# nem0/LumixEngine

Hardware: AMD Instinct MI355X
Metric: entities_culled_per_sec (higher is better)
Workload: dtype f32; 1 GPU; BASELINE config 2: 10000000 static entities per GPU (sparse, cube +-15000), 1 frustum (fov 60, 16:9, near 0.1, far 10000), cull + compaction; entities_per_gpu=10000000, frusta=1, repetitions=1

## Files before the change

lumixengine_amd/build.py:

```python
from __future__ import annotations

import os
import shutil
import subprocess
import sys
from concurrent.futures import ThreadPoolExecutor

PKG = os.path.dirname(os.path.abspath(__file__))
ROOT = os.path.dirname(PKG)
CSRC = os.path.join(PKG, "csrc")
OBJ = os.path.join(PKG, "build")
LIB = os.path.join(PKG, "liblumix_mi355.so")
SOURCES = ["cull_kernels.hip", "xform_kernels.hip", "skin_kernels.hip", "lmx_capi_ctx.hip", "lmx_capi_cull.hip", "lmx_capi_cull_set.hip", "lmx_capi_cull_async.hip", "lmx_capi_cull_results.hip", "lmx_capi_world.hip",
           "lmx_capi_skin.hip", "lmx_capi_exchange.hip", "keys_kernels.hip", "lmx_capi_keys.hip", "anim_kernels.hip", "lmx_capi_anim.hip", "im_kernels.hip", "lmx_capi_im.hip", "draw_kernels.hip", "lmx_capi_draw.hip", "pose_kernels.hip", "lmx_capi_poses.hip", "cluster_kernels.hip", "lmx_capi_clusters.hip", "ray_kernels.hip", "lmx_capi_rays.hip", "ray_scene_kernels.hip", "lmx_capi_rays_scene.hip",
           "lmx_frustum.cpp", "lmx_cluster_planes.cpp", "lmx_world_blob.cpp"]
HEADERS = [os.path.join(CSRC, "lmx_math.h"), os.path.join(CSRC, "lmx_kernels.h"), os.path.join(CSRC, "lmx_cull_layout.h"), os.path.join(CSRC, "lmx_context.h"), os.path.join(CSRC, "lmx_cull_host.h"), os.path.join(CSRC, "lmx_im.h"), os.path.join(CSRC, "lmx_entity_tr.h"), os.path.join(CSRC, "lmx_ray_math.h"), os.path.join(ROOT, "include", "lumix_mi355.h"),
           os.path.join(ROOT, "include", "lmx_types.h")]
FLAGS = ["--offload-arch=gfx950", "-O3", "-std=c++17", "-ffp-contract=off", "-fPIC", "-fvisibility=hidden", "-Wall", "-Wno-unused-function",
         "-I" + os.path.join(ROOT, "include"), "-I" + CSRC] + os.environ.get("LMX_HIPCC_EXTRA", "").split()


def hipcc() -> str:
    exe = shutil.which("hipcc") or "/opt/rocm/bin/hipcc"
    if not os.path.exists(exe):
        raise RuntimeError("hipcc not found: the gfx950 extension cannot be built")
    return exe


def _stale(target: str, deps) -> bool:
    if not os.path.exists(target):
        return True
    t = os.path.getmtime(target)
    return any(os.path.getmtime(d) > t for d in deps)


def _compile(src: str) -> str:
    path = os.path.join(CSRC, src)
    obj = os.path.join(OBJ, os.path.splitext(src)[0] + ".o")
    if _stale(obj, [path] + HEADERS):
        cmd = [hipcc()] + FLAGS + (["-x", "hip"] if src.endswith(".hip") else []) + ["-c", path, "-o", obj]
        r = subprocess.run(cmd, capture_output=True, text=True)
        if r.returncode != 0:
            raise RuntimeError(f"hipcc failed for {src}:\n{r.stdout}\n{r.stderr}")
    return obj


def build(force: bool = False) -> str:
    os.makedirs(OBJ, exist_ok=True)
    if force:
        for f in os.listdir(OBJ):
            os.remove(os.path.join(OBJ, f))
        if os.path.exists(LIB):
            os.remove(LIB)
    with ThreadPoolExecutor(max_workers=len(SOURCES)) as ex:
        objs = list(ex.map(_compile, SOURCES))
# ... 11 lines not shown
```

lumixengine_amd/csrc/cull_kernels.hip:

```cpp
#include <algorithm>
#include <cstddef>
#include <cstdlib>

#include "lmx_kernels.h"
#include <type_traits>

#include <hip/hip_ext.h>

namespace lmx {

namespace {

__device__ __forceinline__ uint32_t lane_id() { return __builtin_amdgcn_mbcnt_hi(~0u, __builtin_amdgcn_mbcnt_lo(~0u, 0u)); }
__device__ __forceinline__ uint32_t mbcnt64(uint64_t mask) {
	return __builtin_amdgcn_mbcnt_hi((uint32_t)(mask >> 32), __builtin_amdgcn_mbcnt_lo((uint32_t)mask, 0u));
}
typedef uint32_t u32x4_a4 __attribute__((ext_vector_type(4), aligned(4)));
__device__ __forceinline__ float readlane_f(float v, int lane) { return __uint_as_float(__builtin_amdgcn_readlane(__float_as_uint(v), lane)); }

struct TileScalars {
	uint32_t ent_begin, cell_cap, n_frusta;
	uint32_t keys_packed;
	uint32_t out_stride, cnt_pad, cnt_frustum_stride, n_zero;
	int32_t* out_slots;
	float pretest_n1s;
};

constexpr int KA_NX = 0, KA_NY = 6, KA_NZ = 12, KA_D = 18, KA_ORIGIN = 44;
static_assert(sizeof(DevFrustum) == 200 && offsetof(DevFrustum, origin) == KA_ORIGIN * 4 && offsetof(DevFrustum, d) == KA_D * 4, "kernarg offsets of DevFrustum");

__device__ __forceinline__ uint32_t tile_status_lanes(const TileBox* box, uint32_t lane) {
	const float* ka = (const float*)__builtin_amdgcn_kernarg_segment_ptr();
	const int32_t* bi = reinterpret_cast<const int32_t*>(box);
	const uint32_t flags = (uint32_t)bi[6];
	const uint32_t a = lane % 3u, kind = (lane / 3u) & 3u;
	const int32_t idx = bi[(kind & 1u) * 3u + a];
	const double org = reinterpret_cast<const double*>(ka + KA_ORIGIN)[a];
	const uint32_t p = (lane & 7u) < 6u ? (lane & 7u) : 5u;
	const float nx = ka[KA_NX + p], ny = ka[KA_NY + p], nz = ka[KA_NZ + p], d = ka[KA_D + p];
	const uint32_t hi = flags << 2;
	if (flags & TILE_EMPTY) return TILE_REJECT | hi;
	if (flags & TILE_HAS_BIG) return TILE_MIXED | hi;
	const double cs = (double)CELL_SIZE;
	const double off = kind == 0u ? -cs : (kind == 3u ? 2 * cs : cs);
	const float val = (float)(cs * idx + off - org);
	const float lx = readlane_f(val, 0), ly = readlane_f(val, 1), lz = readlane_f(val, 2);
	const float hx = readlane_f(val, 3), hy = readlane_f(val, 4), hz = readlane_f(val, 5);
	const float clx = readlane_f(val, 6), cly = readlane_f(val, 7), clz = readlane_f(val, 8);
	const float chx = readlane_f(val, 9), chy = readlane_f(val, 10), chz = readlane_f(val, 11);
	const float b1 = max_f(abs_f(lx), abs_f(chx)) + max_f(abs_f(ly), abs_f(chy)) + max_f(abs_f(lz), abs_f(chz));
	const float n1 = abs_f(nx) + abs_f(ny) + abs_f(nz);
	const float margin = max_f(1.0f, n1) * (2.0f + 4e-6f * b1) + 1e-6f * abs_f(d);
	bool rej, in;
	{
// ... 7 lines not shown
		in = dp > -d + margin;
	}
	const bool plane_lane = lane < 6u;
	if (__ballot(plane_lane && rej) != 0) return TILE_REJECT | hi;
	if (__ballot(plane_lane && !in) == 0) return TILE_ACCEPT | hi;
	bool skip;
	{
		const float bx = nx < 0.0f ? chx : lx, by = ny < 0.0f ? chy : ly, bz = nz < 0.0f ? chz : lz;
		const float dp = (nx * bx) + (ny * by) + (nz * bz);
		skip = dp > -d + margin;
	}
	return TILE_MIXED | hi | (((uint32_t)__ballot(plane_lane && skip) & 63u) << 8);
}

__device__ __forceinline__ uint32_t tile_status_lanes_multi(const TileBox* box, uint32_t lane, int nf, uint32_t* flags_out) {
	const float* ka = (const float*)__builtin_amdgcn_kernarg_segment_ptr();
	const int32_t* bi = reinterpret_cast<const int32_t*>(box);
	const uint32_t flags = (uint32_t)bi[6];
	*flags_out = flags;
	if (flags & TILE_EMPTY) return 0u;
	uint32_t all_mixed = 0;
	for (int f = 0; f < nf; ++f) all_mixed |= (uint32_t)TILE_MIXED << (2 * f);
	if (flags & TILE_HAS_BIG) return all_mixed;
	const uint32_t f = lane / 6u < (uint32_t)nf ? lane / 6u : (uint32_t)nf - 1u, k = lane % 6u;
	const bool plane_lane = lane < (uint32_t)nf * 6u;
	const float* fr = ka + f * (uint32_t)(sizeof(DevFrustum) / sizeof(float));
	const float nx = fr[KA_NX + k], ny = fr[KA_NY + k], nz = fr[KA_NZ + k], d = fr[KA_D + k];
	const double* org = reinterpret_cast<const double*>(fr + KA_ORIGIN);
	const double cs = (double)CELL_SIZE;
	const double ox = org[0], oy = org[1], oz = org[2];
	const float lx = (float)(cs * bi[0] - cs - ox), ly = (float)(cs * bi[1] - cs - oy), lz = (float)(cs * bi[2] - cs - oz);
// ... 44 lines not shown
		t = t + z2 * nz;
		t = t + dd;
		t = t + r2;
		culled = culled || (t.x < 0) || (t.y < 0);
	}
	return !culled;
}


struct alignas(16) CellInfo { float d[6]; uint32_t cls, pad; };
static_assert(sizeof(CellInfo) == 32, "two ds_read_b128 per (lane, chunk, frustum)");

#ifndef LMX_ASM_SGPR
#define LMX_ASM_SGPR(x) "+s"(x)
#endif
#define LMX_CULL_WAVES_ATTR(F) __attribute__((amdgpu_waves_per_eu((F) == 1 ? 1 : 5)))

template <int F, int WAVES, int CHW, int GRP, int FORM, int SLOTS_I>
__global__ __launch_bounds__(WAVES * 64) LMX_CULL_WAVES_ATTR(F) void k_cull_tile(const FrustaArg fr_arg, const float4* __restrict__ g_spheres, const int32_t* __restrict__ g_ids,
	const ChunkHdr* __restrict__ g_hdr, const CellKey* __restrict__ g_tile_cells, const uint32_t* __restrict__ g_tile_tab, const TileBox* __restrict__ g_tile_box,
	const uint2* __restrict__ g_tile_out, int32_t* __restrict__ g_out_ids, uint32_t* __restrict__ g_counts, uint32_t* __restrict__ g_counts_next, const TileScalars a) {
	constexpr bool SLOTS = SLOTS_I != 0;
	constexpr uint32_t TILE = WAVES * CHW * 64;
	constexpr uint32_t THREADS = WAVES * 64;
	constexpr int FS = F == 1 ? 1 : MAX_FRUSTA;
	static_assert(CHW * FS <= 32, "visibility bits of a wave's chunks x frusta live in one register");
	LMX_DYNAMIC_LDS(CellInfo, s_info);
	__shared__ __attribute__((aligned(16))) float s_nrm[F != 1 ? MAX_FRUSTA : 1][F != 1 ? 20 : 4];
	const DevFrustum* __restrict__ frp = (const DevFrustum*)__builtin_amdgcn_kernarg_segment_ptr();
	const int nf = F == 1 ? 1 : (int)a.n_frusta;

	const uint32_t lane = lane_id();
	const uint32_t wave = __builtin_amdgcn_readfirstlane(threadIdx.x >> 6);
	const uint32_t tile_ent = a.ent_begin + blockIdx.x * TILE;
	const uint32_t tile_index = tile_ent / TILE;

	for (uint32_t i = blockIdx.x * THREADS + threadIdx.x; i < a.n_zero; i += gridDim.x * THREADS) g_counts_next[i] = 0;

	uint32_t st_bits = 0, tile_flags = 0, plane_skip = 0;
	bool any_mixed = false, any_live = false;
	if constexpr (FORM != 0) {
		static_assert(F == 1, "the lane-parallel tile test handles one frustum");
		__shared__ uint32_t s_verdict;
		if (wave == 0) {
			const uint32_t v = tile_status_lanes(g_tile_box + tile_index, lane);
			if (lane == 0) s_verdict = v;
		}
		__syncthreads();
		const uint32_t r = s_verdict;
		st_bits = r & 3u;
		tile_flags = (r >> 2) & 63u;
		plane_skip = __builtin_amdgcn_readfirstlane((r >> 8) & 63u);
// ... 7 lines not shown
			if (lane == 0) {
				s_verdict_multi[0] = v;
				s_verdict_multi[1] = fl;
			}
		}
		__syncthreads();
		st_bits = __builtin_amdgcn_readfirstlane(s_verdict_multi[0]);
		tile_flags = __builtin_amdgcn_readfirstlane(s_verdict_multi[1]);
		static_assert(TILE_REJECT == 0 && TILE_ACCEPT == 1 && TILE_MIXED == 2, "the verdicts of all frusta are read off the 2-bit fields by bit logic");
		any_mixed = ((st_bits >> 1) & ~st_bits & 0x5555u) != 0;
		any_live = st_bits != 0;
	}
	if (!any_live) return;
	uint32_t tile_word = 0;
	v2f* s_d2 = reinterpret_cast<v2f*>(s_info);
	uint32_t* s_word = reinterpret_cast<uint32_t*>(s_d2 + (F != 1 ? (size_t)nf * a.cell_cap * 3 : 0));
	constexpr bool SPLIT = F != 1 && WAVES == 4;
	uint16_t* s_w16 = reinterpret_cast<uint16_t*>(s_word);
	if constexpr (F != 1) {
		static_assert(TILE_ACCEPT == 1 && CELL_ACCEPT == 1, "a settled frustum contributes CELL_ACCEPT or nothing: its verdict field IS its class field");
		tile_word = st_bits & ~(st_bits >> 1) & 0x5555u;
	}

	constexpr bool STREAMING = F == 1 && (FORM == 2 || FORM == 4);
	constexpr bool PRELOAD = STREAMING || F != 1;
	typedef float v4f_pre __attribute__((ext_vector_type(4)));
	v4f_pre pre_sp[PRELOAD ? GRP : 1];
	int32_t pre_id[PRELOAD ? GRP : 1];
	auto preload_group0 = [&](auto with_spheres) {
		if constexpr (PRELOAD) {
			const size_t e0 = ((size_t)((tile_ent >> 6) + wave * CHW) << 6) + lane;
#pragma unroll
			for (int i = 0; i < GRP; ++i) {
				pre_id[i] = __builtin_nontemporal_load(g_ids + e0 + i * 64);
				if constexpr (decltype(with_spheres)::value) pre_sp[i] = __builtin_nontemporal_load(reinterpret_cast<const v4f_pre*>(g_spheres + e0 + i * 64));
			}
		}
	};
	uint32_t first_cell = 0;
	if (any_mixed) {
		first_cell = g_tile_tab[2 * tile_index];
		const uint32_t n_cells = g_tile_tab[2 * tile_index + 1];
		const bool packed_keys = F == 1 ? FORM <= 2 : a.keys_packed != 0;
		const char* keys = reinterpret_cast<const char*>(g_tile_cells) + ((size_t)tile_index * a.cell_cap << (packed_keys ? 3 : 4));
		struct FetchedKey { uint4 raw; int32_t lo[3]; };
		auto fetch_key = [&](uint32_t t) -> FetchedKey {
			FetchedKey k;
			if (packed_keys) {
				const uint2 raw = reinterpret_cast<const uint2*>(keys)[t];
				k.raw = uint4{raw.x, raw.y, 0u, 0u};
				uint32_t zero = 0;
				asm volatile("" : "+v"(zero));
				const int32_t* box_lo = reinterpret_cast<const int32_t*>(g_tile_box + tile_index) + zero;
				k.lo[0] = box_lo[0]; k.lo[1] = box_lo[1]; k.lo[2] = box_lo[2];
			} else {
				k.raw = reinterpret_cast<const uint4*>(keys)[t];
				k.lo[0] = k.lo[1] = k.lo[2] = 0;
			}
			return k;
// ... 28 lines not shown
#pragma unroll
						for (int k = 0; k < 6; k += 2) {
							const v2f qx = v2f{frp[f].px[k], frp[f].px[k + 1]} + ox, qy = v2f{frp[f].py[k], frp[f].py[k + 1]} + oy, qz = v2f{frp[f].pz[k], frp[f].pz[k + 1]} + oz;
							v2f t = qx * v2f{frp[f].nx[k], frp[f].nx[k + 1]};
							t = t + qy * v2f{frp[f].ny[k], frp[f].ny[k + 1]};
							t = t + qz * v2f{frp[f].nz[k], frp[f].nz[k + 1]};
							ci.d[k] = -t.x; ci.d[k + 1] = -t.y;
						}
					} else {
#pragma unroll
						for (int k = 0; k < 6; ++k) ci.d[k] = relative_plane_d(frp[f], off, k);
					}
				}
			}
			if constexpr (F != 1) {
				v2f* rec = s_d2 + (size_t)(f * a.cell_cap + t) * 3;
				rec[0] = v2f{ci.d[0], ci.d[1]}; rec[1] = v2f{ci.d[2], ci.d[3]}; rec[2] = v2f{ci.d[4], ci.d[5]};
			} else {
				s_info[f * a.cell_cap + t] = ci;
			}
			return ci.cls;
		};
		if constexpr (F == 1) {
			const FetchedKey fetched0 = fetch_key(threadIdx.x < a.cell_cap ? threadIdx.x : 0u);
			__builtin_amdgcn_sched_barrier(0);
			preload_group0(std::true_type{});
			__builtin_amdgcn_sched_barrier(0);
			CellKey key0 = decode_key(fetched0);
			asm volatile("" : "+v"(key0.ix), "+v"(key0.iy), "+v"(key0.iz), "+v"(key0.meta));
			for (uint32_t t = threadIdx.x; t < n_cells; t += THREADS) classify(t, 0, t == threadIdx.x ? key0 : load_key(t));
		} else {
			const uint32_t t_first = SPLIT ? lane : threadIdx.x, t_step = SPLIT ? 64u : THREADS;
			const FetchedKey fetched0 = fetch_key(t_first < a.cell_cap ? t_first : 0u);
			FetchedKey fetched1 = fetched0;
			if constexpr (SPLIT) fetched1 = fetch_key(t_first + t_step < a.cell_cap ? t_first + t_step : 0u);
			__builtin_amdgcn_sched_barrier(0);
			preload_group0(std::true_type{});
			__builtin_amdgcn_sched_barrier(0);
			const uint32_t my_fields = SPLIT ? 0x0303u << (2u * wave) : 0xffffu;
			for (uint32_t t = t_first; t < n_cells; t += t_step) {
				const CellKey key = t == t_first ? decode_key(fetched0) : (SPLIT && t == t_first + t_step ? decode_key(fetched1) : load_key(t));
				uint32_t word = tile_word & my_fields;
#pragma unroll 1
				for (int f = SPLIT ? (int)wave : 0; f < nf; f += SPLIT ? WAVES : 1) {
					if (((st_bits >> (2 * f)) & 3u) != TILE_MIXED) continue;
					word |= classify(t, f, key) << (2 * f);
				}
				if constexpr (SPLIT) s_w16[4u * t + wave] = (uint16_t)word;
				else s_word[t] = word;
			}
// ... 58 lines not shown
		if (pretest_tile) {
			const uint32_t row = lane & 31u, k = lane >> 5;
			const uint32_t rp = (row & 3u) + 4u * ((row >> 3) & 1u), rh = (row >> 2) & 1u, rq = row >> 4;
#pragma unroll
			for (int gq = 0; gq < NG; ++gq) {
				const uint32_t rf = 4u * gq + 2u * rh + rq;
				const bool row_on = rp < 6u && rf < (uint32_t)nf;
				const uint32_t fs = row_on ? rf : 0u, ps = row_on ? rp : 0u;
				const float nx = row_on ? s_nrm[fs][ps] : 0.f, ny = row_on ? s_nrm[fs][6u + ps] : 0.f, nz = row_on ? s_nrm[fs][12u + ps] : 0.f;
				const uint32_t hi_xy = pk_bf16(nx, ny), hi_z1 = pk_bf16(nz, row_on ? 1.0f : 0.f);
				const uint32_t lo_xy = pk_bf16(nx - __uint_as_float(hi_xy << 16), ny - __uint_as_float(hi_xy & 0xffff0000u)), lo_z0 = pk_bf16(nz - __uint_as_float(hi_z1 << 16), 0.f);
				pre_ab[gq] = k ? u32x4_t{lo_xy, lo_z0, 0u, 0u} : u32x4_t{hi_xy, hi_z1, hi_xy, hi_z1};
#pragma unroll
				for (int q = 0; q < 2; ++q) {
					const uint32_t fl = 4u * gq + 2u * k + q;
					pre_off[gq][q] = (fl < (uint32_t)nf ? fl : (uint32_t)nf - 1u) * a.cell_cap * 3u;
					const uint32_t f_lo = 4u * gq + q, f_hi = f_lo + 2u;
					pre_care[gq][q] = ((mixed_bits >> (2 * f_lo)) & 1u ? 0x00000000ffffffffull : 0ull) | ((mixed_bits >> (2 * f_hi)) & 1u ? 0xffffffff00000000ull : 0ull);
				}
			}
		}
	}

	const uint32_t chunk0 = (tile_ent >> 6) + wave * CHW;
	static_assert(CHW % GRP == 0, "groups tile the wave's chunks");
	int32_t id[CHW];
	uint32_t vis_bits = 0;
	uint32_t mine = 0;
	uint32_t vis2[F != 1 ? CHW : 1];
#pragma unroll
	for (int i = 0; i < (F != 1 ? CHW : 1); ++i) vis2[i] = 0;
// ... 30 lines not shown
			}
		} else {
#pragma unroll
			for (int i = 0; i < GRP; ++i) {
				local[i] = 0;
				cls_word[i] = F != 1 ? tile_word : (uint32_t)CELL_ACCEPT;
			}
		}
#pragma unroll
		for (int i = 0; i < GRP; ++i) {
			const bool lane_live = F != 1 ? cls_word[i] != 0 : (cls_word[i] & 3u) != CELL_REJECT;
			const bool lane_test = F != 1 ? (cls_word[i] & 0xaaaau) != 0  : (cls_word[i] & 3u) == CELL_TEST;
			need_id_bits |= ((uint32_t)__popcll(__ballot(lane_live)) != 0u ? 1u : 0u) << i;
			need_sphere_bits |= ((uint32_t)__popcll(__ballot(lane_test)) != 0u ? 1u : 0u) << i;
		}
#define need_id(i) (((need_id_bits >> (i)) & 1u) != 0)
#define need_sphere(i) (((need_sphere_bits >> (i)) & 1u) != 0)
		float4 sp[GRP];
		typedef float v4f __attribute__((ext_vector_type(4)));
		v4f spv[F != 1 ? GRP : 1];
#pragma unroll
		for (int i = 0; i < GRP; ++i) {
			const uint32_t e = ((chunk0 + g + i) << 6) + lane;
			if constexpr (F != 1) {
				static_assert(F == 1 || GRP == CHW, "one group");
				(void)e;
				id[g + i] = pre_id[i];
				sp[i] = make_float4(pre_sp[i].x, pre_sp[i].y, pre_sp[i].z, pre_sp[i].w);
				continue;
			}
// ... 107 lines not shown
						if (need_sphere(i) && ((exact_chunks >> i) & 1u) && __ballot(((cls_word[i] >> (2 * f)) & 3u) == CELL_TEST) != 0) test_chunks |= 1u << i;
					}
				}
				float4 nq[5];
				if (test_chunks != 0) {
#pragma unroll
					for (int k = 0; k < 5; ++k) nq[k] = reinterpret_cast<const float4*>(s_nrm[f])[k];
				}
				const float* nrm = reinterpret_cast<const float*>(nq);
#pragma unroll
				for (int h = 0; h < GRP; h += 2) {
					float dq[2][6];
					if ((test_chunks >> h) & 3u) {
#pragma unroll
						for (int j = 0; j < 2; ++j) {
							const v2f* rec = s_d2 + (size_t)(f * a.cell_cap + local[h + j]) * 3;
							const v2f d01 = rec[0], d23 = rec[1], d45 = rec[2];
							dq[j][0] = d01.x; dq[j][1] = d01.y; dq[j][2] = d23.x; dq[j][3] = d23.y; dq[j][4] = d45.x; dq[j][5] = d45.y;
						}
					}
#pragma unroll
					for (int j = 0; j < 2; ++j) {
						const int i = h + j;
						uint32_t culled = 0;
						if ((test_chunks >> i) & 1u) {
							asm volatile("" : "+v"(spv[i]));
							const v2f xy = __builtin_shufflevector(spv[i], spv[i], 0, 1), zw = __builtin_shufflevector(spv[i], spv[i], 2, 3);
							const v2f x2 = __builtin_shufflevector(xy, xy, 0, 0), y2 = __builtin_shufflevector(xy, xy, 1, 1);
							const v2f z2 = __builtin_shufflevector(zw, zw, 0, 0), r2 = __builtin_shufflevector(zw, zw, 1, 1);
#pragma unroll
							for (int k = 0; k < 6; k += 2) {
// ... 22 lines not shown
			DevFrustum fn;
			if (need_sphere_bits != 0) {
#pragma unroll
				for (int k = 0; k < 6; ++k) {
					fn.nx[k] = frp[0].nx[k]; fn.ny[k] = frp[0].ny[k]; fn.nz[k] = frp[0].nz[k];
					asm volatile("" : LMX_ASM_SGPR(fn.nx[k]), LMX_ASM_SGPR(fn.ny[k]), LMX_ASM_SGPR(fn.nz[k]));
				}
			}
			static_assert(CELL_REJECT == 0 && CELL_ACCEPT == 1 && CELL_TEST == 2, "class encoding");
#pragma unroll
			for (int h = 0; h < GRP; h += DB) {
				v4f d03[DB];
				v2f d45[DB];
#pragma unroll
				for (int j = 0; j < DB; ++j) {
					const char* ci = reinterpret_cast<const char*>(s_info) + (cls_word[h + j] & ~31u);
					d03[j] = *reinterpret_cast<const v4f*>(ci);
					d45[j] = *reinterpret_cast<const v2f*>(ci + 16);
				}
#pragma unroll
				for (int j = 0; j < DB; ++j) {
					const int i = h + j;
					if (!need_id(i)) continue;
					bool vis = (cls_word[i] & 3u) == CELL_ACCEPT;
					if (need_sphere(i)) {
						const float d[6] = {d03[j].x, d03[j].y, d03[j].z, d03[j].w, d45[j].x, d45[j].y};
						const bool pass = sphere_visible_d_pk(fn, d, sp[i].x, sp[i].y, sp[i].z, sp[i].w);
						vis = vis || ((cls_word[i] & 3u) == CELL_TEST && pass);
					}
					vis = vis && id[g + i] >= 0;
					if constexpr (STAGE) {
						const uint64_t mask = __ballot(vis);
						if (vis) {
							s_stage_ids[wave][staged + mbcnt64(mask)] = id[g + i];
							if constexpr (SLOTS) s_stage_slots[wave][staged + mbcnt64(mask)] = (int32_t)(((chunk0 + g + i) << 6) + lane);
						}
						staged += (uint32_t)__popcll(mask);
					} else {
						const uint32_t c = (uint32_t)__popcll(__ballot(vis));
						mine += lane == 0u ? c : 0u;
						vis_bits |= (vis ? 1u : 0u) << ((g + i) * FS);
					}
				}
// ... 47 lines not shown
		if (__builtin_amdgcn_readlane(mine, f) == 0) continue;
		uint32_t run = __builtin_amdgcn_readlane(base_v, f) + win;
		int32_t* dst = g_out_ids + (size_t)f * a.out_stride;
#pragma unroll
		for (int i = 0; i < CHW; ++i) {
			const bool v = F != 1 ? ((vis2[F != 1 ? i : 0] >> (2 * f)) & 1u) != 0 : ((vis_bits >> (i * FS + f)) & 1u) != 0;
			const uint64_t mask = __ballot(v);
			if (v) dst[run + mbcnt64(mask)] = id[i];
			if constexpr (SLOTS) {
				if (v) (a.out_slots + (size_t)f * a.out_stride)[run + mbcnt64(mask)] = (int32_t)(((chunk0 + i) << 6) + lane);
			}
			run += (uint32_t)__popcll(mask);
		}
	}
}

constexpr int DYN_THREADS = 256;

template <int TILE>
__global__ __launch_bounds__(DYN_THREADS) void k_cull_dynamic(const double* __restrict__ px, const double* __restrict__ py,
	const double* __restrict__ pz, const float* __restrict__ radius, const int32_t* __restrict__ ids, FrustaArg fr, int n_frusta,
	TypeTable dyn_tt, uint32_t slot_begin, CullOut out) {
	LMX_DYNAMIC_LDS(int32_t, s_stage);
	uint32_t* s_cnt = reinterpret_cast<uint32_t*>(s_stage + n_frusta * TILE);
	uint32_t* s_base = s_cnt + MAX_FRUSTA;
	const uint32_t lane = lane_id();
	const uint32_t block_slot = slot_begin + blockIdx.x * (uint32_t)TILE;
	uint32_t type = 0;
#pragma unroll
	for (int t = 0; t < MAX_TYPES; ++t) {
// ... 113 lines not shown
	uint32_t dst_stride, uint32_t dst_cap, const int32_t* __restrict__ src2 ,
	int32_t* __restrict__ dst2) {
	const uint32_t s = blockIdx.x, f = blockIdx.y;
	const uint32_t c = counts[f * cnt_frustum_stride + s * cnt_pad];
	const size_t from_at = (size_t)f * src_stride + win_base[s];
	const uint32_t at = type_start[f * type_start_stride + shard_type[s]] + pref[f * n_shards + s];
	const size_t to_at = (size_t)f * dst_stride + at;
	const uint32_t room = at < dst_cap ? dst_cap - at : 0u;
	const uint32_t n = c < room ? c : room;
	for (uint32_t k = blockIdx.z * 256u + threadIdx.x; k < n; k += gridDim.z * 256u) {
		dst[to_at + k] = src[from_at + k];
		if (src2 != nullptr) dst2[to_at + k] = src2[from_at + k];
	}
}

__global__ __launch_bounds__(256) void k_cull_pack(const int32_t* __restrict__ src, const uint32_t* __restrict__ win_base, const uint32_t* __restrict__ counts,
	uint32_t cnt_pad, const uint8_t* __restrict__ shard_type, uint32_t n_shards, int32_t* __restrict__ rec_base, PackLayout lay,
	uint32_t src_stride, uint32_t cnt_stride) {
	__shared__ uint32_t s_part[4];
	__shared__ uint32_t s_tot[MAX_TYPES];
	const uint32_t s = blockIdx.x, t = threadIdx.x;
	src += (size_t)blockIdx.z * src_stride;
	counts += (size_t)blockIdx.z * cnt_stride;
	uint32_t* const header = reinterpret_cast<uint32_t*>(rec_base + lay.off[blockIdx.z]);
	int32_t* const dst = rec_base + lay.off[blockIdx.z] + MAX_TYPES;
	const uint32_t dst_cap = lay.cap[blockIdx.z];
	const bool totals_block = s == 0 && blockIdx.y == 0;
	const uint32_t c = counts[s * cnt_pad];
	if (blockIdx.y * 256u >= c && !totals_block) return;
	const int32_t* from = src + win_base[s];
	const uint32_t k0 = blockIdx.y * 256u + t;
	const int32_t first = k0 < c ? from[k0] : 0;
	uint32_t before = 0;
// ... 20 lines not shown
hipError_t tile_f(hipStream_t s, const CullDeviceView& v, uint32_t ent_begin, uint32_t ent_end, const TypeTable& tt, const FrustaArg& fr, int n_frusta,
	const CullOut& out) {
	constexpr uint32_t TILE = WAVES * CHW * 64;
	static_assert(TILE_ALIGN % TILE == 0, "tiles must not straddle type ranges");
	constexpr int K = TILE == 4096 ? 0 : (TILE == 2048 ? 1 : 2);
	const uint32_t tiles = (ent_end - ent_begin) / TILE;
	if (!tiles) {
		if (out.ev_start != nullptr) {
			(void)hipEventRecord(out.ev_start, s);
			(void)hipEventRecord(out.ev_stop, s);
		}
		return hipSuccess;
	}
	TileScalars a;
	(void)tt;
	a.ent_begin = ent_begin;
	a.cell_cap = v.tile_cap[K];
	a.keys_packed = v.keys_packed ? 1u : 0u;
	a.n_frusta = (uint32_t)n_frusta;
	a.out_stride = out.stride;
	a.cnt_pad = out.cnt_pad;
	a.cnt_frustum_stride = out.cnt_frustum_stride;
	a.n_zero = out.n_zero;
	a.out_slots = out.slots;
	{
		float n1 = 0.f;
		bool finite = true;
		for (int f = 0; f < n_frusta; ++f) {
			for (int k = 0; k < 6; ++k) {
				const float v = (__builtin_fabsf(fr.f[f].nx[k]) + __builtin_fabsf(fr.f[f].ny[k])) + __builtin_fabsf(fr.f[f].nz[k]);
				finite = finite && v <= 3.0e38f;
				n1 = v > n1 ? v : n1;
			}
		}
		a.pretest_n1s = finite ? n1 * 1.000001f * 134217728.0f : __builtin_inff();
	}
	if (out.ev_start != nullptr)
		hipExtLaunchKernelGGL((k_cull_tile<F, WAVES, CHW, GRP, FORM, SLOTS_I>), dim3(tiles), dim3(WAVES * 64), cull_tile_lds_bytes(n_frusta, a.cell_cap), s, out.ev_start, out.ev_stop, 0, fr,
			v.spheres, v.ids, v.hdr, v.tile_cells[K], v.tile_tab[K], v.tile_box[K], v.tile_out[K], out.ids, out.counts, out.counts_next, a);
	else
		hipLaunchKernelGGL((k_cull_tile<F, WAVES, CHW, GRP, FORM, SLOTS_I>), dim3(tiles), dim3(WAVES * 64), cull_tile_lds_bytes(n_frusta, a.cell_cap), s, fr, v.spheres, v.ids, v.hdr,
			v.tile_cells[K], v.tile_tab[K], v.tile_box[K], v.tile_out[K], out.ids, out.counts, out.counts_next, a);
	return hipGetLastError();
}

}

size_t cull_tile_lds_bytes(int n_frusta, uint32_t cell_cap) {
	return n_frusta > 1 ? (size_t)n_frusta * cell_cap * 24 + (size_t)cell_cap * (n_frusta > 4 ? 8 : 4) : (size_t)cell_cap * sizeof(CellInfo);
}

uint32_t cull_tile_size(int n_frusta, int variant) {
	(void)variant;
	return n_frusta <= 4 ? 2048u : 1024u;
}

hipError_t launch_cull_tile(hipStream_t s, const CullDeviceView& v, uint32_t ent_begin, uint32_t ent_end, const TypeTable& tt, const FrustaArg& fr,
// ... 79 lines not shown
		shard_type, type_start, type_start_stride, pref, n_shards, dst, dst_stride, dst_cap, src2, dst2);
	return hipGetLastError();
}

hipError_t launch_cull_pack_layout(hipStream_t s, const int32_t* src, const uint32_t* win_base, const uint32_t* counts, uint32_t cnt_pad, const uint8_t* shard_type,
	uint32_t n_shards, uint32_t max_shard_cap, int32_t* rec_base, const PackLayout& lay, uint32_t n_frusta, uint32_t src_stride, uint32_t cnt_stride) {
	if (!n_frusta) return hipSuccess;
	if (n_frusta > (uint32_t)MAX_FRUSTA) return hipErrorInvalidValue;
	if (!n_shards) {
		for (uint32_t f = 0; f < n_frusta; ++f)
			if (hipError_t e = hipMemsetAsync(rec_base + lay.off[f], 0, MAX_TYPES * sizeof(uint32_t), s)) return e;
		return hipSuccess;
	}
	if (n_shards > (uint32_t)FIN_MAX_SHARDS) return hipErrorInvalidValue;
	const uint32_t splits = std::max(1u, std::min(64u, max_shard_cap / 4096u));
	hipLaunchKernelGGL(k_cull_pack, dim3(n_shards, splits, n_frusta), dim3(256), 0, s, src, win_base, counts, cnt_pad, shard_type, n_shards, rec_base, lay, src_stride,
		cnt_stride);
	return hipGetLastError();
}

hipError_t launch_cull_pack(hipStream_t s, const int32_t* src, const uint32_t* win_base, const uint32_t* counts, uint32_t cnt_pad, const uint8_t* shard_type,
	uint32_t n_shards, uint32_t max_shard_cap, uint32_t* header, int32_t* dst, uint32_t dst_cap, uint32_t n_frusta, uint32_t src_stride, uint32_t cnt_stride,
	uint32_t rec_stride) {
	if (n_frusta > (uint32_t)MAX_FRUSTA || dst != reinterpret_cast<int32_t*>(header) + MAX_TYPES) return hipErrorInvalidValue;
	PackLayout lay = {};
	for (uint32_t f = 0; f < n_frusta; ++f) {
		lay.off[f] = (uint64_t)f * rec_stride;
		lay.cap[f] = dst_cap;
	}
	return launch_cull_pack_layout(s, src, win_base, counts, cnt_pad, shard_type, n_shards, max_shard_cap, reinterpret_cast<int32_t*>(header), lay, n_frusta, src_stride, cnt_stride);
}

// ... 2 lines not shown
```

lumixengine_amd/csrc/lmx_capi_cull.hip:

```cpp
#include "lmx_cull_host.h"

#include <optional>

using namespace lmx;

namespace {

static_assert(sizeof(LayoutSphere) == sizeof(float4) && sizeof(LayoutCell) == sizeof(CellKey) && sizeof(LayoutChunkHdr) == sizeof(ChunkHdr), "layout PODs mirror the device types");
static_assert(LAYOUT_MAX_TYPES == MAX_TYPES && LAYOUT_CHUNK == CHUNK && LAYOUT_TILE_ALIGN == TILE_ALIGN && LAYOUT_CELL_DEAD == CELL_DEAD, "layout constants");

constexpr uint32_t DYN_ALIGN = 2048;
constexpr uint32_t DYN_MAX_SHARDS = 8;

CullDeviceView static_view(const CullSet& cs) {
	CullDeviceView v;
	v.spheres = cs.spheres.p;
	v.ids = cs.ids.p;
	v.hdr = cs.hdr.p;
	v.n_padded = cs.n_padded;
	v.keys_packed = cs.keys_packed;
	for (int k = 0; k < 3; ++k) {
		v.tile_cells[k] = cs.tile_cells[k].p;
		v.tile_tab[k] = cs.tile_tab[k].p;
		v.tile_box[k] = cs.tile_box[k].p;
// ... 587 lines not shown
```

lumixengine_amd/csrc/lmx_kernels.h:

```cpp
#pragma once

#include <hip/hip_runtime.h>
#include <stdint.h>

#include "lmx_math.h"
#include "lmx_types.h"

#ifndef LMX_DYNAMIC_LDS
#define LMX_DYNAMIC_LDS(T, name) extern __shared__ T name[]
#endif

namespace lmx {

constexpr int MAX_FRUSTA = 8;
constexpr int MAX_TYPES = 8;
constexpr uint32_t CHUNK = 64;
constexpr uint32_t TILE_ALIGN = 4096;
constexpr uint32_t CELL_DEAD = 0x80000000u;

struct CellKey { int32_t ix, iy, iz; uint32_t meta; };
struct PackedCellKey { uint32_t xy, zf; };
constexpr uint32_t PACKED_CELL_BIG = 1u << 16, PACKED_CELL_DEAD = 1u << 31;
struct ChunkHdr { uint32_t cell, pad; uint64_t flags; };

struct TypeTable {
	uint32_t ent_start[MAX_TYPES];
	uint32_t ent_end[MAX_TYPES];
	uint32_t shard_first[MAX_TYPES];
	uint32_t shard_n[MAX_TYPES];
};

struct FrustaArg { DevFrustum f[MAX_FRUSTA]; };

// ... 429 lines not shown
```

Baseline: 785.0 billion entities/s.

## Reorder cull kernel arguments for kernarg preload and pack cell classes

Reorders k_cull_tile parameters so the pointers and scalars used first come before the frusta, and enables kernarg preloading of the first six arguments for the cull kernels. This aims to cut scalar load latency at kernel start. It also packs pairs of 16-bit cell class words into one register for the single-frustum path and raises waves_per_eu for some single-frustum forms, trading register pressure for occupancy. Asm barriers force certain loads into vector registers, and static_asserts check the new kernarg layout.

```diff
diff --git a/lumixengine_amd/build.py b/lumixengine_amd/build.py
--- a/lumixengine_amd/build.py
+++ b/lumixengine_amd/build.py
@@ -18,6 +18,7 @@
            os.path.join(ROOT, "include", "lmx_types.h")]
 FLAGS = ["--offload-arch=gfx950", "-O3", "-std=c++17", "-ffp-contract=off", "-fPIC", "-fvisibility=hidden", "-Wall", "-Wno-unused-function",
          "-I" + os.path.join(ROOT, "include"), "-I" + CSRC] + os.environ.get("LMX_HIPCC_EXTRA", "").split()
+SOURCE_FLAGS = {"cull_kernels.hip": ["-mllvm", "-amdgpu-kernarg-preload-count=6"]}
 
 
 def hipcc() -> str:
@@ -38,7 +39,7 @@
     path = os.path.join(CSRC, src)
     obj = os.path.join(OBJ, os.path.splitext(src)[0] + ".o")
     if _stale(obj, [path] + HEADERS):
-        cmd = [hipcc()] + FLAGS + (["-x", "hip"] if src.endswith(".hip") else []) + ["-c", path, "-o", obj]
+        cmd = [hipcc()] + FLAGS + SOURCE_FLAGS.get(src, []) + (["-x", "hip"] if src.endswith(".hip") else []) + ["-c", path, "-o", obj]
         r = subprocess.run(cmd, capture_output=True, text=True)
         if r.returncode != 0:
             raise RuntimeError(f"hipcc failed for {src}:\n{r.stdout}\n{r.stderr}")
diff --git a/lumixengine_amd/csrc/cull_kernels.hip b/lumixengine_amd/csrc/cull_kernels.hip
--- a/lumixengine_amd/csrc/cull_kernels.hip
+++ b/lumixengine_amd/csrc/cull_kernels.hip
@@ -19,25 +19,46 @@
 __device__ __forceinline__ float readlane_f(float v, int lane) { return __uint_as_float(__builtin_amdgcn_readlane(__float_as_uint(v), lane)); }
 
 struct TileScalars {
-	uint32_t ent_begin, cell_cap, n_frusta;
+	int32_t* out_slots;
+	uint32_t n_frusta;
 	uint32_t keys_packed;
-	uint32_t out_stride, cnt_pad, cnt_frustum_stride, n_zero;
-	int32_t* out_slots;
+	uint32_t out_stride, cnt_pad, cnt_frustum_stride;
 	float pretest_n1s;
 };
+static_assert(sizeof(TileScalars) == 32, "with it the arguments in front of the frusta fill exactly one 128-byte line");
+
+struct CullTileKernargs {
+	const TileBox* g_tile_box; uint32_t ent_begin, n_zero; uint32_t* g_counts_next;
+	const uint32_t* g_tile_tab; const CellKey* g_tile_cells; const ChunkHdr* g_hdr; uint32_t cell_cap;
+	const float4* g_spheres; const int32_t* g_ids; const uint2* g_tile_out; int32_t* g_out_ids; uint32_t* g_counts; TileScalars a;
+	FrustaArg fr_arg;
+};
+constexpr size_t KA_FRUSTA_BYTES = offsetof(CullTileKernargs, fr_arg);
+static_assert(KA_FRUSTA_BYTES == 128 && KA_FRUSTA_BYTES % alignof(double) == 0, "the frusta's place in k_cull_tile's kernarg segment (fp64 origins)");
+template <typename T, typename... A> constexpr size_t kernarg_offset_of(void (*)(A...)) {
+	size_t off = 0, found = ~(size_t)0;
+	((off = (off + (alignof(A) > 16 ? 16 : alignof(A)) - 1) / (alignof(A) > 16 ? 16 : alignof(A)) * (alignof(A) > 16 ? 16 : alignof(A)),
+	  found = (found == ~(size_t)0 && std::is_same<typename std::remove_cv<A>::type, T>::value) ? off : found, off += sizeof(A)), ...);
+	return found;
+}
 
 constexpr int KA_NX = 0, KA_NY = 6, KA_NZ = 12, KA_D = 18, KA_ORIGIN = 44;
 static_assert(sizeof(DevFrustum) == 200 && offsetof(DevFrustum, origin) == KA_ORIGIN * 4 && offsetof(DevFrustum, d) == KA_D * 4, "kernarg offsets of DevFrustum");
+__device__ __forceinline__ const float* kernarg_frusta() { return reinterpret_cast<const float*>((const char*)__builtin_amdgcn_kernarg_segment_ptr() + KA_FRUSTA_BYTES); }
 
 __device__ __forceinline__ uint32_t tile_status_lanes(const TileBox* box, uint32_t lane) {
-	const float* ka = (const float*)__builtin_amdgcn_kernarg_segment_ptr();
+	const float* ka = kernarg_frusta();
 	const int32_t* bi = reinterpret_cast<const int32_t*>(box);
-	const uint32_t flags = (uint32_t)bi[6];
 	const uint32_t a = lane % 3u, kind = (lane / 3u) & 3u;
-	const int32_t idx = bi[(kind & 1u) * 3u + a];
-	const double org = reinterpret_cast<const double*>(ka + KA_ORIGIN)[a];
+	uint32_t zero = 0;
+	asm volatile("" : "+v"(zero));
+	uint32_t flags_v = (uint32_t)bi[6u + zero];
+	int32_t idx = bi[(kind & 1u) * 3u + a];
+	double org = reinterpret_cast<const double*>(ka + KA_ORIGIN)[a];
 	const uint32_t p = (lane & 7u) < 6u ? (lane & 7u) : 5u;
-	const float nx = ka[KA_NX + p], ny = ka[KA_NY + p], nz = ka[KA_NZ + p], d = ka[KA_D + p];
+	float nx = ka[KA_NX + p], ny = ka[KA_NY + p], nz = ka[KA_NZ + p], d = ka[KA_D + p];
+	asm volatile("" : "+v"(flags_v), "+v"(idx), "+v"(org), "+v"(nx), "+v"(ny), "+v"(nz), "+v"(d));
+	const uint32_t flags = __builtin_amdgcn_readfirstlane(flags_v);
 	const uint32_t hi = flags << 2;
 	if (flags & TILE_EMPTY) return TILE_REJECT | hi;
 	if (flags & TILE_HAS_BIG) return TILE_MIXED | hi;
@@ -75,7 +96,7 @@
 }
 
 __device__ __forceinline__ uint32_t tile_status_lanes_multi(const TileBox* box, uint32_t lane, int nf, uint32_t* flags_out) {
-	const float* ka = (const float*)__builtin_amdgcn_kernarg_segment_ptr();
+	const float* ka = kernarg_frusta();
 	const int32_t* bi = reinterpret_cast<const int32_t*>(box);
 	const uint32_t flags = (uint32_t)bi[6];
 	*flags_out = flags;
@@ -150,12 +171,13 @@
 #ifndef LMX_ASM_SGPR
 #define LMX_ASM_SGPR(x) "+s"(x)
 #endif
-#define LMX_CULL_WAVES_ATTR(F) __attribute__((amdgpu_waves_per_eu((F) == 1 ? 1 : 5)))
+#define LMX_CULL_WAVES_ATTR(F, FORM) __attribute__((amdgpu_waves_per_eu((F) != 1 ? 5 : ((FORM) == 1 || (FORM) == 3 ? 8 : 1))))
 
 template <int F, int WAVES, int CHW, int GRP, int FORM, int SLOTS_I>
-__global__ __launch_bounds__(WAVES * 64) LMX_CULL_WAVES_ATTR(F) void k_cull_tile(const FrustaArg fr_arg, const float4* __restrict__ g_spheres, const int32_t* __restrict__ g_ids,
-	const ChunkHdr* __restrict__ g_hdr, const CellKey* __restrict__ g_tile_cells, const uint32_t* __restrict__ g_tile_tab, const TileBox* __restrict__ g_tile_box,
-	const uint2* __restrict__ g_tile_out, int32_t* __restrict__ g_out_ids, uint32_t* __restrict__ g_counts, uint32_t* __restrict__ g_counts_next, const TileScalars a) {
+__global__ __launch_bounds__(WAVES * 64) LMX_CULL_WAVES_ATTR(F, FORM) void k_cull_tile(const TileBox* __restrict__ g_tile_box, const uint32_t ent_begin, const uint32_t n_zero, uint32_t* __restrict__ g_counts_next,
+	const uint32_t* __restrict__ g_tile_tab, const CellKey* __restrict__ g_tile_cells, const ChunkHdr* __restrict__ g_hdr, const uint32_t cell_cap,
+	const float4* __restrict__ g_spheres, const int32_t* __restrict__ g_ids, const uint2* __restrict__ g_tile_out, int32_t* __restrict__ g_out_ids, uint32_t* __restrict__ g_counts,
+	const TileScalars a, const FrustaArg fr_arg) {
 	constexpr bool SLOTS = SLOTS_I != 0;
 	constexpr uint32_t TILE = WAVES * CHW * 64;
 	constexpr uint32_t THREADS = WAVES * 64;
@@ -163,15 +185,16 @@
 	static_assert(CHW * FS <= 32, "visibility bits of a wave's chunks x frusta live in one register");
 	LMX_DYNAMIC_LDS(CellInfo, s_info);
 	__shared__ __attribute__((aligned(16))) float s_nrm[F != 1 ? MAX_FRUSTA : 1][F != 1 ? 20 : 4];
-	const DevFrustum* __restrict__ frp = (const DevFrustum*)__builtin_amdgcn_kernarg_segment_ptr();
+	const DevFrustum* __restrict__ frp = reinterpret_cast<const DevFrustum*>(kernarg_frusta());
 	const int nf = F == 1 ? 1 : (int)a.n_frusta;
 
 	const uint32_t lane = lane_id();
 	const uint32_t wave = __builtin_amdgcn_readfirstlane(threadIdx.x >> 6);
-	const uint32_t tile_ent = a.ent_begin + blockIdx.x * TILE;
+	uint32_t tile_ent = ent_begin + blockIdx.x * TILE;
+	asm volatile("" : LMX_ASM_SGPR(tile_ent));
 	const uint32_t tile_index = tile_ent / TILE;
 
-	for (uint32_t i = blockIdx.x * THREADS + threadIdx.x; i < a.n_zero; i += gridDim.x * THREADS) g_counts_next[i] = 0;
+	for (uint32_t i = blockIdx.x * THREADS + threadIdx.x; i < n_zero; i += gridDim.x * THREADS) g_counts_next[i] = 0;
 
 	uint32_t st_bits = 0, tile_flags = 0, plane_skip = 0;
 	bool any_mixed = false, any_live = false;
@@ -209,7 +232,7 @@
 	if (!any_live) return;
 	uint32_t tile_word = 0;
 	v2f* s_d2 = reinterpret_cast<v2f*>(s_info);
-	uint32_t* s_word = reinterpret_cast<uint32_t*>(s_d2 + (F != 1 ? (size_t)nf * a.cell_cap * 3 : 0));
+	uint32_t* s_word = reinterpret_cast<uint32_t*>(s_d2 + (F != 1 ? (size_t)nf * cell_cap * 3 : 0));
 	constexpr bool SPLIT = F != 1 && WAVES == 4;
 	uint16_t* s_w16 = reinterpret_cast<uint16_t*>(s_word);
 	if constexpr (F != 1) {
@@ -237,7 +260,7 @@
 		first_cell = g_tile_tab[2 * tile_index];
 		const uint32_t n_cells = g_tile_tab[2 * tile_index + 1];
 		const bool packed_keys = F == 1 ? FORM <= 2 : a.keys_packed != 0;
-		const char* keys = reinterpret_cast<const char*>(g_tile_cells) + ((size_t)tile_index * a.cell_cap << (packed_keys ? 3 : 4));
+		const char* keys = reinterpret_cast<const char*>(g_tile_cells) + ((size_t)tile_index * cell_cap << (packed_keys ? 3 : 4));
 		struct FetchedKey { uint4 raw; int32_t lo[3]; };
 		auto fetch_key = [&](uint32_t t) -> FetchedKey {
 			FetchedKey k;
@@ -296,15 +319,15 @@
 				}
 			}
 			if constexpr (F != 1) {
-				v2f* rec = s_d2 + (size_t)(f * a.cell_cap + t) * 3;
+				v2f* rec = s_d2 + (size_t)(f * cell_cap + t) * 3;
 				rec[0] = v2f{ci.d[0], ci.d[1]}; rec[1] = v2f{ci.d[2], ci.d[3]}; rec[2] = v2f{ci.d[4], ci.d[5]};
 			} else {
-				s_info[f * a.cell_cap + t] = ci;
+				s_info[f * cell_cap + t] = ci;
 			}
 			return ci.cls;
 		};
 		if constexpr (F == 1) {
-			const FetchedKey fetched0 = fetch_key(threadIdx.x < a.cell_cap ? threadIdx.x : 0u);
+			const FetchedKey fetched0 = fetch_key(threadIdx.x < cell_cap ? threadIdx.x : 0u);
 			__builtin_amdgcn_sched_barrier(0);
 			preload_group0(std::true_type{});
 			__builtin_amdgcn_sched_barrier(0);
@@ -313,9 +336,9 @@
 			for (uint32_t t = threadIdx.x; t < n_cells; t += THREADS) classify(t, 0, t == threadIdx.x ? key0 : load_key(t));
 		} else {
 			const uint32_t t_first = SPLIT ? lane : threadIdx.x, t_step = SPLIT ? 64u : THREADS;
-			const FetchedKey fetched0 = fetch_key(t_first < a.cell_cap ? t_first : 0u);
+			const FetchedKey fetched0 = fetch_key(t_first < cell_cap ? t_first : 0u);
 			FetchedKey fetched1 = fetched0;
-			if constexpr (SPLIT) fetched1 = fetch_key(t_first + t_step < a.cell_cap ? t_first + t_step : 0u);
+			if constexpr (SPLIT) fetched1 = fetch_key(t_first + t_step < cell_cap ? t_first + t_step : 0u);
 			__builtin_amdgcn_sched_barrier(0);
 			preload_group0(std::true_type{});
 			__builtin_amdgcn_sched_barrier(0);
@@ -404,7 +427,7 @@
 #pragma unroll
 				for (int q = 0; q < 2; ++q) {
 					const uint32_t fl = 4u * gq + 2u * k + q;
-					pre_off[gq][q] = (fl < (uint32_t)nf ? fl : (uint32_t)nf - 1u) * a.cell_cap * 3u;
+					pre_off[gq][q] = (fl < (uint32_t)nf ? fl : (uint32_t)nf - 1u) * cell_cap * 3u;
 					const uint32_t f_lo = 4u * gq + q, f_hi = f_lo + 2u;
 					pre_care[gq][q] = ((mixed_bits >> (2 * f_lo)) & 1u ? 0x00000000ffffffffull : 0ull) | ((mixed_bits >> (2 * f_hi)) & 1u ? 0xffffffff00000000ull : 0ull);
 				}
@@ -465,6 +488,17 @@
 			need_id_bits |= ((uint32_t)__popcll(__ballot(lane_live)) != 0u ? 1u : 0u) << i;
 			need_sphere_bits |= ((uint32_t)__popcll(__ballot(lane_test)) != 0u ? 1u : 0u) << i;
 		}
+		constexpr bool PACK_CLS = F == 1 && GRP == CHW;
+		uint32_t cls_pair[PACK_CLS ? GRP / 2 : 1];
+		if constexpr (PACK_CLS) {
+			static_assert(TILE / 1024u * MAX_CELLS_PER_1024 * 32u <= 0x10000u, "a 2048-sphere tile's record offsets fit 16 bits next to the class");
+#pragma unroll
+			for (int j = 0; j < GRP / 2; ++j) {
+				cls_pair[j] = cls_word[2 * j] | (cls_word[2 * j + 1] << 16);
+				asm volatile("" : "+v"(cls_pair[j]));
+			}
+		}
+		auto cw = [&](int i) -> uint32_t { return PACK_CLS ? (cls_pair[PACK_CLS ? i >> 1 : 0] >> (16 * (i & 1))) & 0xffffu : cls_word[i]; };
 #define need_id(i) (((need_id_bits >> (i)) & 1u) != 0)
 #define need_sphere(i) (((need_sphere_bits >> (i)) & 1u) != 0)
 		float4 sp[GRP];
@@ -602,7 +636,7 @@
 					if ((test_chunks >> h) & 3u) {
 #pragma unroll
 						for (int j = 0; j < 2; ++j) {
-							const v2f* rec = s_d2 + (size_t)(f * a.cell_cap + local[h + j]) * 3;
+							const v2f* rec = s_d2 + (size_t)(f * cell_cap + local[h + j]) * 3;
 							const v2f d01 = rec[0], d23 = rec[1], d45 = rec[2];
 							dq[j][0] = d01.x; dq[j][1] = d01.y; dq[j][2] = d23.x; dq[j][3] = d23.y; dq[j][4] = d45.x; dq[j][5] = d45.y;
 						}
@@ -655,7 +689,7 @@
 				v2f d45[DB];
 #pragma unroll
 				for (int j = 0; j < DB; ++j) {
-					const char* ci = reinterpret_cast<const char*>(s_info) + (cls_word[h + j] & ~31u);
+					const char* ci = reinterpret_cast<const char*>(s_info) + (cw(h + j) & ~31u);
 					d03[j] = *reinterpret_cast<const v4f*>(ci);
 					d45[j] = *reinterpret_cast<const v2f*>(ci + 16);
 				}
@@ -663,11 +697,11 @@
 				for (int j = 0; j < DB; ++j) {
 					const int i = h + j;
 					if (!need_id(i)) continue;
-					bool vis = (cls_word[i] & 3u) == CELL_ACCEPT;
+					bool vis = (cw(i) & 3u) == CELL_ACCEPT;
 					if (need_sphere(i)) {
 						const float d[6] = {d03[j].x, d03[j].y, d03[j].z, d03[j].w, d45[j].x, d45[j].y};
 						const bool pass = sphere_visible_d_pk(fn, d, sp[i].x, sp[i].y, sp[i].z, sp[i].w);
-						vis = vis || ((cls_word[i] & 3u) == CELL_TEST && pass);
+						vis = vis || ((cw(i) & 3u) == CELL_TEST && pass);
 					}
 					vis = vis && id[g + i] >= 0;
 					if constexpr (STAGE) {
@@ -745,6 +779,9 @@
 		}
 	}
 }
+
+static_assert(kernarg_offset_of<FrustaArg>(static_cast<decltype(&k_cull_tile<1, 4, 8, 8, 1, 0>)>(nullptr)) == KA_FRUSTA_BYTES, "k_cull_tile's parameters and CullTileKernargs differ");
+static_assert(kernarg_offset_of<FrustaArg>(static_cast<decltype(&k_cull_tile<0, 4, 4, 4, 0, 0>)>(nullptr)) == KA_FRUSTA_BYTES, "k_cull_tile's parameters and CullTileKernargs differ");
 
 constexpr int DYN_THREADS = 256;
 
@@ -888,9 +925,9 @@
 	}
 }
 
-__global__ __launch_bounds__(256) void k_cull_pack(const int32_t* __restrict__ src, const uint32_t* __restrict__ win_base, const uint32_t* __restrict__ counts,
-	uint32_t cnt_pad, const uint8_t* __restrict__ shard_type, uint32_t n_shards, int32_t* __restrict__ rec_base, PackLayout lay,
-	uint32_t src_stride, uint32_t cnt_stride) {
+__global__ __launch_bounds__(256) void k_cull_pack(const uint32_t* __restrict__ counts, const uint32_t* __restrict__ win_base, const int32_t* __restrict__ src,
+	uint32_t cnt_pad, uint32_t cnt_stride, uint32_t src_stride, uint32_t n_shards, const uint8_t* __restrict__ shard_type, int32_t* __restrict__ rec_base,
+	PackLayout lay) {
 	__shared__ uint32_t s_part[4];
 	__shared__ uint32_t s_tot[MAX_TYPES];
 	const uint32_t s = blockIdx.x, t = threadIdx.x;
@@ -941,14 +978,12 @@
 	}
 	TileScalars a;
 	(void)tt;
-	a.ent_begin = ent_begin;
-	a.cell_cap = v.tile_cap[K];
+	const uint32_t cell_cap = v.tile_cap[K];
 	a.keys_packed = v.keys_packed ? 1u : 0u;
 	a.n_frusta = (uint32_t)n_frusta;
 	a.out_stride = out.stride;
 	a.cnt_pad = out.cnt_pad;
 	a.cnt_frustum_stride = out.cnt_frustum_stride;
-	a.n_zero = out.n_zero;
 	a.out_slots = out.slots;
 	{
 		float n1 = 0.f;
@@ -963,11 +998,11 @@
 		a.pretest_n1s = finite ? n1 * 1.000001f * 134217728.0f : __builtin_inff();
 	}
 	if (out.ev_start != nullptr)
-		hipExtLaunchKernelGGL((k_cull_tile<F, WAVES, CHW, GRP, FORM, SLOTS_I>), dim3(tiles), dim3(WAVES * 64), cull_tile_lds_bytes(n_frusta, a.cell_cap), s, out.ev_start, out.ev_stop, 0, fr,
-			v.spheres, v.ids, v.hdr, v.tile_cells[K], v.tile_tab[K], v.tile_box[K], v.tile_out[K], out.ids, out.counts, out.counts_next, a);
+		hipExtLaunchKernelGGL((k_cull_tile<F, WAVES, CHW, GRP, FORM, SLOTS_I>), dim3(tiles), dim3(WAVES * 64), cull_tile_lds_bytes(n_frusta, cell_cap), s, out.ev_start, out.ev_stop, 0,
+			v.tile_box[K], ent_begin, out.n_zero, out.counts_next, v.tile_tab[K], v.tile_cells[K], v.hdr, cell_cap, v.spheres, v.ids, v.tile_out[K], out.ids, out.counts, a, fr);
 	else
-		hipLaunchKernelGGL((k_cull_tile<F, WAVES, CHW, GRP, FORM, SLOTS_I>), dim3(tiles), dim3(WAVES * 64), cull_tile_lds_bytes(n_frusta, a.cell_cap), s, fr, v.spheres, v.ids, v.hdr,
-			v.tile_cells[K], v.tile_tab[K], v.tile_box[K], v.tile_out[K], out.ids, out.counts, out.counts_next, a);
+		hipLaunchKernelGGL((k_cull_tile<F, WAVES, CHW, GRP, FORM, SLOTS_I>), dim3(tiles), dim3(WAVES * 64), cull_tile_lds_bytes(n_frusta, cell_cap), s, v.tile_box[K], ent_begin, out.n_zero,
+			out.counts_next, v.tile_tab[K], v.tile_cells[K], v.hdr, cell_cap, v.spheres, v.ids, v.tile_out[K], out.ids, out.counts, a, fr);
 	return hipGetLastError();
 }
 
@@ -1077,8 +1112,8 @@
 	}
 	if (n_shards > (uint32_t)FIN_MAX_SHARDS) return hipErrorInvalidValue;
 	const uint32_t splits = std::max(1u, std::min(64u, max_shard_cap / 4096u));
-	hipLaunchKernelGGL(k_cull_pack, dim3(n_shards, splits, n_frusta), dim3(256), 0, s, src, win_base, counts, cnt_pad, shard_type, n_shards, rec_base, lay, src_stride,
-		cnt_stride);
+	hipLaunchKernelGGL(k_cull_pack, dim3(n_shards, splits, n_frusta), dim3(256), 0, s, counts, win_base, src, cnt_pad, cnt_stride, src_stride, n_shards, shard_type, rec_base,
+		lay);
 	return hipGetLastError();
 }
 
diff --git a/lumixengine_amd/csrc/lmx_capi_cull.hip b/lumixengine_amd/csrc/lmx_capi_cull.hip
--- a/lumixengine_amd/csrc/lmx_capi_cull.hip
+++ b/lumixengine_amd/csrc/lmx_capi_cull.hip
@@ -8,6 +8,7 @@
 
 static_assert(sizeof(LayoutSphere) == sizeof(float4) && sizeof(LayoutCell) == sizeof(CellKey) && sizeof(LayoutChunkHdr) == sizeof(ChunkHdr), "layout PODs mirror the device types");
 static_assert(LAYOUT_MAX_TYPES == MAX_TYPES && LAYOUT_CHUNK == CHUNK && LAYOUT_TILE_ALIGN == TILE_ALIGN && LAYOUT_CELL_DEAD == CELL_DEAD, "layout constants");
+static_assert(LAYOUT_CELL_BLOCK == 1024 && LAYOUT_MAX_CELLS_PER_BLOCK == MAX_CELLS_PER_1024, "layout constants");
 
 constexpr uint32_t DYN_ALIGN = 2048;
 constexpr uint32_t DYN_MAX_SHARDS = 8;
diff --git a/lumixengine_amd/csrc/lmx_kernels.h b/lumixengine_amd/csrc/lmx_kernels.h
--- a/lumixengine_amd/csrc/lmx_kernels.h
+++ b/lumixengine_amd/csrc/lmx_kernels.h
@@ -17,6 +17,7 @@
 constexpr uint32_t CHUNK = 64;
 constexpr uint32_t TILE_ALIGN = 4096;
 constexpr uint32_t CELL_DEAD = 0x80000000u;
+constexpr uint32_t MAX_CELLS_PER_1024 = 240;
 
 struct CellKey { int32_t ix, iy, iz; uint32_t meta; };
 struct PackedCellKey { uint32_t xy, zf; };
```

Measured after the change: 810.5 billion entities/s, median of 4. +3.3%, better.
